# Chuanming-Liu/DAzimSurfTomo

Hardware: AMD Instinct MI355X
Metric: FMM traveltime fields/sec (256^2 grid, 16 periods) + LSQR SpMV HBM GB/s (higher is better)
Workload: dtype f32

## Files before the change

### dazimsurftomo_amd/__init__.py

```python
import ctypes as C

import numpy as np

from . import _lib
from ._lib import Geom, RefBox, build, load

RMAX = 129
PI_F32 = np.float32(3.1415926535898)


DAZIM_OK, DAZIM_E_SOURCE_OUTSIDE, DAZIM_E_RECEIVER_OUTSIDE, DAZIM_E_NNZ_OVERFLOW, DAZIM_E_BAD_ARG, DAZIM_E_ROOT_NOT_FOUND = 0, 1, 2, 4, 5, 6


class DazimError(RuntimeError):
    def __init__(self, code, msg):
        super().__init__(f"dazim error {code}: {msg}")
        self.code = code


def _is_torch(x):
    return type(x).__module__.startswith("torch")


def _ptr(x, dtype=None):
# ... 157 lines not shown
        kmax = len(tRc)
        if _is_torch(vel):
            import torch
            if lsen is None:
                lsen = torch.empty((nz - 1, kmax, nx * ny), dtype=torch.float32, device=vel.device)
        else:
            vel = np.ascontiguousarray(vel, np.float32)
            pv = np.ascontiguousarray(pv, np.float64)
            if lsen is None:
                lsen = np.zeros((nz - 1, kmax, nx * ny), np.float32)
        fn = self.lib.dazim_ti_kernels_sharded if sharded else self.lib.dazim_ti_kernels
        rc = fn(self._h, nx, ny, nz, _ptr(vel, np.float32), _ptr(depz), C.c_float(minthk), kmax, _ptr(tRc), _ptr(pv), _ptr(lsen))
        self._check(rc)
        return lsen

    def fmm_batch(self, nx, ny, goxd, gozd, dvxd, dvzd, pv, scx, scz, period_idx,
                  veln=None, ttn=None, ttnr=None, nstsr=None, boxes=None, status=None,
                  want_refined=True, keep_fields=False):
        g = geometry(nx, ny, goxd, gozd, dvxd, dvzd)
        kmax = pv.shape[0]
        nfield = int(scx.shape[0])
        if not _is_torch(pv):
            pv = np.ascontiguousarray(pv, np.float64)
            scx = np.ascontiguousarray(scx, np.float32)
            scz = np.ascontiguousarray(scz, np.float32)
            period_idx = np.ascontiguousarray(period_idx, np.int32)
            if ttn is None and not keep_fields:
                ttn = np.zeros((nfield, g.nnx, g.nnz), np.float32)
            if veln is None:
                veln = np.zeros((kmax, g.nnx, g.nnz), np.float32)
            if want_refined and ttnr is None:
                ttnr = np.zeros((nfield, RMAX, RMAX), np.float32)
                nstsr = np.zeros((nfield, RMAX, RMAX), np.int32)
            if boxes is None:
                boxes = (RefBox * max(nfield, 1))()
            if status is None:
                status = np.zeros(nfield, np.int32)
        if keep_fields:
            ttn = None
        bptr = None
        if boxes is not None:
            bptr = C.c_void_p(boxes.data_ptr()) if _is_torch(boxes) else C.cast(boxes, C.c_void_p)
        rc = self.lib.dazim_fmm_batch(self._h, nx, ny, C.c_float(goxd), C.c_float(gozd), C.c_float(dvxd),
                                      C.c_float(dvzd), kmax, _ptr(pv), nfield, _ptr(scx), _ptr(scz),
                                      _ptr(period_idx), _ptr(veln), _ptr(ttn), _ptr(ttnr), _ptr(nstsr),
                                      bptr, _ptr(status))
        out = dict(geom=g, veln=veln, ttn=ttn, ttnr=ttnr, nstsr=nstsr, boxes=boxes, status=status, rc=rc)
        if rc:
            err = DazimError(rc, self.lib.dazim_last_error(self._h).decode())
            err.partial = out
            raise err
        return out

    def rays_build_G(self, nx, ny, goxd, gozd, dvxd, dvzd, vels, fields, scx, scz, period_idx, field_of_ray,
                     rcx, rcz, sen, kernel_idx=None, tpred=None, lsen=None):
        nz = vels.shape[0]
        kmax = fields["veln"].shape[0]
        nfield = int(scx.shape[0])
        nray = int(rcx.shape[0])
        if tpred is None:
            if _is_torch(rcx):
                import torch
                tpred = torch.empty(nray, dtype=torch.float32, device=rcx.device)
            else:
                tpred = np.zeros(nray, np.float32)
        boxes = fields["boxes"]
        bptr = C.c_void_p(boxes.data_ptr()) if _is_torch(boxes) else C.cast(boxes, C.c_void_p)
        h = C.c_void_p()
        nnz = C.c_int64(0)
        nb = C.c_int(0)
        args = [self._h, nx, ny, nz, C.c_float(goxd), C.c_float(gozd), C.c_float(dvxd),
                C.c_float(dvzd), kmax, _ptr(vels, np.float32), nfield, _ptr(scx), _ptr(scz),
                _ptr(period_idx), _ptr(kernel_idx), _ptr(fields["veln"]), _ptr(fields["ttn"]),
                _ptr(fields["ttnr"]), _ptr(fields["nstsr"]), bptr, C.c_int64(nray),
                _ptr(field_of_ray), _ptr(rcx), _ptr(rcz), _ptr(sen[0]), _ptr(sen[1]), _ptr(sen[2])]
        tail = [_ptr(tpred), C.byref(h), C.byref(nnz), C.byref(nb)]
        if lsen is None:
            rc = self.lib.dazim_rays_build_G(*args, *tail)
        else:
            rc = self.lib.dazim_rays_build_G_joint(*args, _ptr(lsen, np.float32), *tail)
        self._check(rc)
        n = (nx - 2) * (ny - 2) * (nz - 1) * (1 if lsen is None else 3)
        return SparseMatrix(self, h, nray, n, nnz.value), tpred, nb.value

    def rays_build_G_maps(self, nx, ny, goxd, gozd, dvxd, dvzd, fields, scx, scz, period_idx, field_of_ray, rcx, rcz,
                          azim=False, tpred=None):
        kmax = fields["veln"].shape[0]
        nfield = int(scx.shape[0])
        nray = int(rcx.shape[0])
        if tpred is None:
            if _is_torch(rcx):
                import torch
                tpred = torch.empty(nray, dtype=torch.float32, device=rcx.device)
            else:
                tpred = np.zeros(nray, np.float32)
        boxes = fields["boxes"]
        bptr = C.c_void_p(boxes.data_ptr()) if _is_torch(boxes) else C.cast(boxes, C.c_void_p)
        h = C.c_void_p()
        nnz = C.c_int64(0)
        nb = C.c_int(0)
        rc = self.lib.dazim_rays_build_G_maps(self._h, nx, ny, C.c_float(goxd), C.c_float(gozd), C.c_float(dvxd), C.c_float(dvzd),
                                              kmax, int(bool(azim)), nfield, _ptr(scx), _ptr(scz), _ptr(period_idx),
                                              _ptr(fields["veln"]), _ptr(fields["ttn"]), _ptr(fields["ttnr"]), _ptr(fields["nstsr"]),
                                              bptr, C.c_int64(nray), _ptr(field_of_ray), _ptr(rcx), _ptr(rcz), _ptr(tpred),
                                              C.byref(h), C.byref(nnz), C.byref(nb))
        self._check(rc)
        n = (nx - 2) * (ny - 2) * kmax * (3 if azim else 1)
        return SparseMatrix(self, h, nray, n, nnz.value), tpred, nb.value

    def phase_map_update(self, nx, ny, pv, dm, minc, maxc, azim):
        kmax = pv.shape[0]
        assert pv.size == kmax * nx * ny and pv.flags.c_contiguous
        ncell = (nx - 2) * (ny - 2)
        nblock = 3 if azim else 1
        assert pv.dtype == np.float64 and dm.dtype == np.float32 and len(dm) == ncell * kmax * nblock
        a1 = np.zeros((kmax, ny - 2, nx - 2), np.float32) if azim else None
        a2 = np.zeros((kmax, ny - 2, nx - 2), np.float32) if azim else None
        st = np.zeros((nblock, kmax, 3), np.float32)
        self._check(self.lib.dazim_phase_map_update(self._h, nx, ny, kmax, int(bool(azim)), _ptr(pv), _ptr(dm), C.c_float(minc),
                                                    C.c_float(maxc), _ptr(a1), _ptr(a2), _ptr(st)))
        return a1, a2, st

    def vs_kernels(self, vel, sen, skern=None):
        nz, ny, nx = vel.shape
        kmax = sen[0].shape[1]
        if skern is None:
            if _is_torch(vel):
                import torch
                skern = torch.empty((nz, kmax, nx * ny), dtype=torch.float64, device=vel.device)
            else:
                skern = np.zeros((nz, kmax, nx * ny), np.float64)
        if not _is_torch(vel):
            vel = np.ascontiguousarray(vel, np.float32)
            sen = [np.ascontiguousarray(s, np.float64) for s in sen]
        self._check(self.lib.dazim_vs_kernels(self._h, nx, ny, nz, kmax, _ptr(vel, np.float32), _ptr(sen[0], np.float64),
                                              _ptr(sen[1], np.float64), _ptr(sen[2], np.float64), _ptr(skern, np.float64)))
        return skern

    def column_lsq(self, nx, ny, nlay, kern, rhs, wdat=None, smooth=0.0, damp=0.0, x=None):
        kmax = kern.shape[1]
        nrhs = rhs.shape[0]
        fp32 = str(kern.dtype).endswith("float32")
        if x is None:
            if _is_torch(rhs):
                import torch
                x = torch.empty((nrhs, nlay, ny - 2, nx - 2), dtype=torch.float32, device=rhs.device)
            else:
                x = np.zeros((nrhs, nlay, ny - 2, nx - 2), np.float32)
        if not _is_torch(rhs):
            kern = np.ascontiguousarray(kern)
            rhs = np.ascontiguousarray(rhs, np.float32)
            wdat = None if wdat is None else np.ascontiguousarray(wdat, np.float32)
        ne = C.c_int(0)
        st = np.zeros((nrhs, kmax, 2), np.float32)
        self._check(self.lib.dazim_column_lsq(self._h, nx, ny, int(nlay), kmax, int(fp32), _ptr(kern, np.float32 if fp32 else np.float64),
                                              nrhs, _ptr(rhs, np.float32), _ptr(wdat, np.float32), C.c_float(smooth), C.c_float(damp),
                                              _ptr(x, np.float32), C.byref(ne), _ptr(st)))
        return x, ne.value, st

# ... 264 lines not shown
```

### dazimsurftomo_amd/csrc/rays.hip

```cpp
#include <cmath>
#include <chrono>
#include <unistd.h>

#include "dazim_internal.h"

#include <rocprim/device/device_scan.hpp>
#include <rocprim/device/device_radix_sort.hpp>

namespace {

#ifdef DZ_RAYS_MARK
#define RAYS_MARK(i) asm volatile("; MARK " #i ::: "memory")
#else
#define RAYS_MARK(i)
#endif

constexpr int GDX = 5, GDZ = 5;
constexpr int RM = DAZIM_RMAX;
constexpr float EARTH = 6371.0f;
constexpr float FTOL = 1e-4f;

struct RayArgs {
  dazim_geom g;
  int nx, ny, nz, kmax;
// ... 151 lines not shown
    }
  return biv;
}

__global__ void k_row_kernels(long n, int kmax, long ncol, const float *__restrict__ vels, const double *__restrict__ svs,
                              const double *__restrict__ svp, const double *__restrict__ srho, double *__restrict__ out) {
  const long i = (long)blockIdx.x * blockDim.x + threadIdx.x;
  if (i >= n) return;
  const long k = i / (kmax * ncol), c = i % ncol;
  out[i] = dz_row_kernel(vels[k * ncol + c], svs[i], svp[i], srho[i]);
}

__global__ void k_ray_keys(long nray, const int *__restrict__ field, const float *__restrict__ scx, const float *__restrict__ scz,
                           const float *__restrict__ rcx, const float *__restrict__ rcz, float inv_dmax, int dbits,
                           unsigned *__restrict__ keys, unsigned *__restrict__ iota, const int *__restrict__ order) {
  const long i = (long)blockIdx.x * blockDim.x + threadIdx.x;
  if (i >= nray) return;
  const int f = field[i];
  const float dx = scx[f] - rcx[i], dz = (scz[f] - rcz[i]) * __sinf(rcx[i]);
  const float d = sqrtf(dx * dx + dz * dz) * inv_dmax;
  const unsigned dmaxq = (1u << dbits) - 1u;
  unsigned q = d >= 1.0f ? dmaxq : (unsigned)(d * (float)dmaxq);
  keys[i] = ((unsigned)(order ? order[f] : f) << dbits) | (dmaxq - q);
  iota[i] = (unsigned)i;
}

constexpr int GP_COUNT = 8, GP_EMIT = 16;
constexpr int RAYS_MINW = 4;
constexpr int RPW_MAX = 64 / GP_COUNT;
__device__ __forceinline__ void cbar() { asm volatile("" ::: "memory"); }

template <bool EMIT, bool AZIM, bool TILED, bool MAP>
__global__ __launch_bounds__(64, AZIM ? 2 : RAYS_MINW) void rays_kernel(RayArgs A_) {
  using ArgP = const __attribute__((address_space(4))) RayArgs *;
  auto launder = [](ArgP p) {
    int z;
    asm volatile("v_mov_b32 %0, 0" : "=v"(z));
    return (ArgP)((const __attribute__((address_space(4))) char *)p + __builtin_amdgcn_readfirstlane(z));
  };
  ArgP Ap = launder((ArgP)__builtin_amdgcn_kernarg_segment_ptr());
#define A (*Ap)
#define RAYS_ARGS_FRESH Ap = launder(Ap)
  constexpr int GP = EMIT ? GP_EMIT : GP_COUNT;
  constexpr int RPW = 64 / GP;
  constexpr int LPR = 16 / GP;
  constexpr int LSTEP = 4 / LPR;
  constexpr unsigned GMASK = (1u << GP) - 1u;
  extern __shared__ __attribute__((aligned(16))) unsigned short s_lists[];
  dazim_geom g;
  g.nvx = A.g.nvx; g.nvz = A.g.nvz; g.nnx = A.g.nnx; g.nnz = A.g.nnz;
  g.gox = A.g.gox; g.goz = A.g.goz; g.dnx = A.g.dnx; g.dnz = A.g.dnz; g.dvx = A.g.dvx; g.dvz = A.g.dvz;
  const int lane = threadIdx.x, grp = lane / GP, gl = lane & (GP - 1);
  const int lm = gl & 3, l0 = gl >> 2;
  const int nnx = g.nnx, nnz = g.nnz, nvx = g.nvx, nvz = g.nvz, ldf = nvz + 2, nf = ldf * (nvx + 2);
  constexpr int NG = AZIM ? 3 : 1;
  const unsigned nvx_magic = A.nvx_magic;
  const int LC = A.lcap;
  unsigned short *s_list = s_lists + (size_t)grp * LC;
  float *gfdm = A.fdm_scratch + ((size_t)blockIdx.x * RPW + grp) * nf * NG;
  float *gfdmc = gfdm + nf, *gfdms = gfdm + 2 * nf;
  const float gox = g.gox, goz = g.goz, dnx = g.dnx, dnz = g.dnz, dvx = g.dvx, dvz = g.dvz;
  const double rdnx = A.r_dnx, rdnz = A.r_dnz, rdnxr = A.r_dnxr, rdnzr = A.r_dnzr, rdvx = A.r_dvx, rdvz = A.r_dvz;
  const unsigned gmask_shift = grp * GP;
  const long nquad = (A.nray + RPW - 1) / RPW;
  const int nxcd = (gridDim.x % 8 == 0) ? 8 : 1;
  unsigned *qcnt = A.qcount + (EMIT ? 8 : 0);
  int chunk = (int)(blockIdx.x % nxcd);
  int traced = 0;
  for (;;) {
    RAYS_ARGS_FRESH;
    long quad = -1;
    if (lane == 0) {
      for (int tried = 0; tried < nxcd; tried++) {
        const long lo = nquad * chunk / nxcd, hi = nquad * (chunk + 1) / nxcd;
        const long b = lo < hi ? (long)atomicAdd(&qcnt[chunk], 1u) : hi;
        if (lo + b < hi) {
          quad = lo + b;
          break;
        }
        if (!EMIT && A.sweeps > 1 && lo < hi && b < (hi - lo) * A.sweeps) {
          quad = lo + b % (hi - lo);
          break;
        }
        chunk = (chunk + 1) % nxcd;
      }
    }
    quad = ((long)__shfl((int)(quad >> 32), 0) << 32) | (unsigned)__shfl((int)quad, 0);
    chunk = __shfl(chunk, 0);
    if (quad < 0) break;
    const long slot = quad * RPW + grp;
    if (!EMIT && A.defer_mark) {
      if (!A.defer_mark[quad]) continue;
      if (A.fdone) {
        const int fq = slot < A.nray ? A.field[A.perm ? (long)A.perm[slot] : slot] : -1;
        const int st = fq >= 0 ? __hip_atomic_load(A.fdone + fq, __ATOMIC_ACQUIRE, __HIP_MEMORY_SCOPE_AGENT) : 1;
        if (__ballot(st != 1) != 0) continue;
        __builtin_amdgcn_fence(__ATOMIC_ACQUIRE, "agent");
      }
      if (A.max_quads > 0 && traced >= A.max_quads) break;
      int mine = 0;
      if (lane == 0) mine = __hip_atomic_exchange(A.defer_mark + quad, 0, __ATOMIC_RELAXED, __HIP_MEMORY_SCOPE_AGENT);
      mine = __shfl(mine, 0);
      if (!mine) continue;
      traced++;
      if (lane == 0) atomicAdd(&A.qcount[18], 1u);
    }
    if (slot >= A.nray) continue;
    const long ray = A.perm ? (long)A.perm[slot] : slot;
    const int f = A.field[ray];
    const float scx = A.scx[f], scz = A.scz[f], rcx = A.rcx[ray], rcz = A.rcz[ray];
    const float *veln = A.veln + (size_t)(A.period[f] - 1) * nnx * nnz;
    const float *ttn = TILED ? A.ttn + (size_t)(A.tslot ? A.tslot[f] : f) * A.fstride : A.ttn + (size_t)f * nnx * nnz;
    const int tsh = TILED ? A.tsh : 0;
    auto tnode = [&](int x0, int z0) -> float {
      return TILED ? ttn[dz_tile_x(x0, tsh) + dz_tile_z(z0)] : ttn[(size_t)x0 * nnz + z0];
    };
    const float *ttnr = A.ttnr + (size_t)f * RM * RM;
    const int *nstsr = A.nstsr + (size_t)f * RM * RM;
    const dazim_refbox bx = A.boxes[f];
    const int saved = EMIT ? A.nlist[ray] : -1;
    if (saved < 0)
      for (int i = gl; i < nf * NG; i += GP) gfdm[i] = 0.0f;
    cbar();
    int status = 0, rb = 0;
    if (!EMIT) {
      int irx = (int)divr(rcx - gox, rdnx) + 1, irz = (int)divr(rcz - goz, rdnz) + 1;
      if (irx < 1 || irx > nnx || irz < 1 || irz > nnz) status = DAZIM_E_RECEIVER_OUTSIDE;
      if (!status) {
        if (irx == nnx) irx--;
        if (irz == nnz) irz--;
        const int isx = (int)divr(scx - gox, rdnx) + 1, isz = (int)divr(scz - goz, rdnz) + 1;
        float sred = ((scx - rcx) * EARTH) * ((scx - rcx) * EARTH);
        const float e2 = (scz - rcz) * EARTH * dz_sinf(rcx);
        sred = sqrtf(sred + e2 * e2);
        bool sw = sred < A.dplh;
        if (isx == irx && isz == irz) sw = true;
        float trr;
        if (sw) {
          const float vs = bilin_cell(g, veln, isx, isz, scx, scz, rdnx, rdnz);
          const float vr = bilin_cell(g, veln, irx, irz, rcx, rcz, rdnx, rdnz);
          trr = 2.0f * sred / (vs + vr);
        } else {
          const float drx = (rcx - gox) - (float)(irx - 1) * dnx;
          const float drz = (rcz - goz) - (float)(irz - 1) * dnz;
          trr = 0.0f;
#pragma unroll
          for (int k = 1; k <= 2; k++)
#pragma unroll
            for (int l = 1; l <= 2; l++) {
              const float produ = (1.0f - fabsf(divr((float)(l - 1) * dnz - drz, rdnz))) *
                                  (1.0f - fabsf(divr((float)(k - 1) * dnx - drx, rdnx)));
              trr = trr + tnode(irx - 2 + k, irz - 2 + l) * produ;
            }
        }
        if (gl == 0) A.dsurf[ray] = trr;
      }
    }
    const float goxr = bx.goxr, gozr = bx.gozr, dnxr = bx.dnxr, dnzr = bx.dnzr;
    const int nnxr = bx.nnxr, nnzr = bx.nnzr;
    const int isx = (int)divr(scx - goxr, rdnxr) + 1, isz = (int)divr(scz - gozr, rdnzr) + 1;
    const float dpl = 0.5f * A.dplh;
    int ipx = (int)divr(rcx - gox, rdnx) + 1, ipz = (int)divr(rcz - goz, rdnz) + 1;
    if (ipx < 1 || ipx >= nnx || ipz < 1 || ipz >= nnz) status = DAZIM_E_RECEIVER_OUTSIDE;
    if (!status && saved < 0) {
      float x0 = rcx, z0 = rcz;
      float sinx0 = dz_sinf(x0);
      int sw = 0;
      float sred = ((scx - x0) * EARTH) * ((scx - x0) * EARTH);
      float e2 = (scz - z0) * EARTH * sinx0;
      sred = sqrtf(sred + e2 * e2);
      if (sred < 2.0f * dpl) sw = 1;
      int ipxr = (int)divr(rcx - goxr, rdnxr) + 1, ipzr = (int)divr(rcz - gozr, rdnzr) + 1;
      auto in_refined = [&](int px, int pz) -> int {
        if (px < 1 || px >= nnxr || pz < 1 || pz >= nnzr) return 0;
        const int *sp = nstsr + (size_t)(px - 1) * RM + (pz - 1);
        if (sp[0] != 0 || sp[1] != 0) return 0;
        if (sp[RM] != 0 || sp[RM + 1] != 0) return 0;
        return 1;
      };
      int igref = in_refined(ipxr, ipzr);
      if (sw == 0 && igref == 1 && ipxr == isx && ipzr == isz) sw = 1;
      const bool keep_pts = !EMIT && A.pts != nullptr && gl == 0;
      float2 *rp = A.pts ? A.pts + (size_t)ray * A.pcap : nullptr;
      int np = 1;
      if (keep_pts) {
        rp[0] = make_float2(rcx, rcz);
        if (sw == 1) { if (A.pcap > 1) rp[1] = make_float2(scx, scz); np = 2; }
      }
      int cbx = -100, cbz = -100;
      float acc[LPR], accc[LPR], accs[LPR];
#pragma unroll
      for (int q = 0; q < LPR; q++) acc[q] = accc[q] = accs[q] = 0.0f;
      auto flush = [&]() {
        if (cbx > -100) {
#pragma unroll
          for (int q = 0; q < LPR; q++) {
            const int fi = (cbx + lm) * ldf + (cbz + l0 + q * LSTEP);
            gfdm[fi] = acc[q];
            if (AZIM) { gfdmc[fi] = accc[q]; gfdms[fi] = accs[q]; }
          }
        }
      };
      float tc00, tc01, tc10, tc11, tr00 = 0.0f, tr01 = 0.0f, tr10 = 0.0f, tr11 = 0.0f;
      auto load_corner_times = [&]() {
        if (TILED) {
          const int x0 = dz_tile_x(ipx - 1, tsh), x1 = dz_tile_x(ipx, tsh), z0 = dz_tile_z(ipz - 1), z1 = dz_tile_z(ipz);
          tc00 = ttn[x0 + z0]; tc01 = ttn[x0 + z1]; tc10 = ttn[x1 + z0]; tc11 = ttn[x1 + z1];
        } else {
          const float *t = ttn + (size_t)(ipx - 1) * nnz + (ipz - 1);
          tc00 = t[0]; tc01 = t[1]; tc10 = t[nnz]; tc11 = t[nnz + 1];
        }
      };
      auto load_refined_corner_times = [&]() {
        if (ipxr >= 1 && ipxr < nnxr && ipzr >= 1 && ipzr < nnzr) {
          const float *u = ttnr + (size_t)(ipxr - 1) * RM + (ipzr - 1);
          tr00 = u[0]; tr01 = u[1]; tr10 = u[RM]; tr11 = u[RM + 1];
        }
      };
      load_corner_times();
      load_refined_corner_times();
      bool carry = false;
      float rdc[LPR];
#pragma unroll
      for (int q = 0; q < LPR; q++) rdc[q] = 0.0f;
      float fart = __builtin_inff();
      int nnx_in = 0, nnz_in = 0;
      const long maxrp = (long)nnx * nnz;
      for (long j = 1; j <= maxrp; j++) {
        if (sw == 1) break;
        RAYS_MARK(0);
        float dtx, dtz;
        if (igref == 1) {
          dtx = tr10 - tr00;
          dtx = dtx + tr11 - tr01;
          dtx = divr(dtx, A.r_e2dnxr);
          dtz = tr01 - tr00;
          dtz = dtz + tr11 - tr10;
          dtz = dtz / (2.0f * EARTH * sinx0 * dnzr);
        } else {
          dtx = tc10 - tc00;
          dtx = dtx + tc11 - tc01;
          dtx = divr(dtx, A.r_e2dnx);
          dtz = tc01 - tc00;
          dtz = dtz + tc11 - tc10;
          dtz = dtz / (2.0f * EARTH * sinx0 * dnz);
        }
        const float rd1 = sqrtf(dtx * dtx + dtz * dtz);
        float x1 = x0 - dpl * dtx / (EARTH * rd1);
        float z1 = z0 - dpl * dtz / (EARTH * sinx0 * rd1);
        RAYS_MARK(1);
// ... 72 lines not shown
        RAYS_MARK(6);
        float drx, drz;
        if (__builtin_expect(__ballot(!carry) != 0, 0)) {
          drx = (x0 - gox) - (float)(ipxo - 1) * dnx;
          drz = (z0 - goz) - (float)(ipzo - 1) * dnz;
          const float vel = vel_at(g, veln, ipxo, ipzo, drx, drz, rdnx, rdnz);
          drx = (x0 - gox) - (float)(ivxo - 1) * dvx;
          drz = (z0 - goz) - (float)(ivzo - 1) * dvz;
          const float vi = basis1(divr(drx, rdvx), lm);
#pragma unroll
          for (int q = 0; q < LPR; q++) rdc[q] = vi * basis1(divr(drz, rdvz), l0 + q * LSTEP) / (vel * vel);
          if (A.plain_step == 0) {
            fart = (float)((RM - 1) / 8 + 1) * fmaxf(dnx, dnz);
            nnx_in = nnx;
            nnz_in = nnz;
          }
        }
        RAYS_MARK(7);
        int ivxt = ivxo, ivzt = ivzo;
        bool endsame = false;
        for (int k = 1; k <= nhp; k++) {
          if (k > 1) {
            const int cp = (k == 2) ? chp0 : chp1;
            if (cp == 1) ivxt = ivx;
            else if (cp == 2) ivzt = ivz;
          }
          const float vrk = (k == 1) ? vr0 : (k == 2 ? vr1 : vr2);
          const float vrp = (k == 2) ? vr0 : vr1;
          const float rigz = z0 + vrk * (z1 - z0);
          const float rigx = x0 + vrk * (x1 - x0);
          const int ipxt = (int)divr(rigx - gox, rdnx) + 1, ipzt = (int)divr(rigz - goz, rdnz) + 1;
          endsame = rigx == x1 && rigz == z1 && ipxt == ipx && ipzt == ipz && ivxt == ivx && ivzt == ivz;
          drx = (rigx - gox) - (float)(ipxt - 1) * dnx;
          drz = (rigz - goz) - (float)(ipzt - 1) * dnz;
          const bool inner = ipxt >= 1 && ipxt < nnx_in && ipzt >= 1 && ipzt < nnz_in;
          endsame = endsame && inner;
          float vel;
          if (__builtin_expect(__ballot(!inner) == 0, 1)) vel = vel_at_interior(g, veln, ipxt, ipzt, drx, drz, rdnx, rdnz);
          else vel = vel_at(g, veln, ipxt, ipzt, drx, drz, rdnx, rdnz);
          drx = (rigx - gox) - (float)(ivxt - 1) * dvx;
          drz = (rigz - goz) - (float)(ivzt - 1) * dvz;
          const float vi = basis1(divr(drx, rdvx), lm);
          float wi[LPR];
#pragma unroll
          for (int q = 0; q < LPR; q++) wi[q] = basis1(divr(drz, rdvz), l0 + q * LSTEP);
          const float dinc = (k == 1) ? vrk * dpl : (vrk - vrp) * dpl;
          const int nbx = ivxt - 1, nbz = ivzt - 1;
          RAYS_MARK(8);
          if (nbx != cbx || nbz != cbz) {
            flush();
            cbar();
            cbx = nbx;
            cbz = nbz;
#pragma unroll
            for (int q = 0; q < LPR; q++) {
              const int fi = (cbx + lm) * ldf + (cbz + l0 + q * LSTEP);
              acc[q] = gfdm[fi];
              if (AZIM) { accc[q] = gfdmc[fi]; accs[q] = gfdms[fi]; }
            }
          }
          RAYS_MARK(9);
#pragma unroll
          for (int q = 0; q < LPR; q++) {
            const float rdc1 = vi * wi[q] / (vel * vel);
            const float rdc2 = rdc[q];
            rdc[q] = rdc1;
            float r1 = -(rdc1 + rdc2) * dinc / 2.0f;
            acc[q] = r1 + acc[q];
            if (AZIM) {
              r1 = -(rdc1 * c2psi + rdc2 * c2psi) * dinc / 2.0f;
              accc[q] = r1 + accc[q];
              r1 = -(rdc1 * s2psi + rdc2 * s2psi) * dinc / 2.0f;
              accs[q] = r1 + accs[q];
            }
          }
        }
        RAYS_MARK(10);
        carry = endsame;
        x0 = x1;
        z0 = z1;
        sinx0 = sinx1;
      RAYS_MARK(11);
      }
      flush();
      if (keep_pts) A.npts[ray] = np <= A.pcap ? np : -1;
    }
    cbar();
    if (!EMIT && gl == 0) {
      if (A.pts && status) A.npts[ray] = 0;
      A.status[ray] = status;
      A.rbflag[ray] = rb;
    }
    int nlist = 0;
    if (saved >= 0) {
      nlist = saved;
      const size_t o = (size_t)ray * A.LK, ov = o * NG;
      for (int i = gl; i < nlist; i += GP) {
        const int c = A.lcell[o + i];
        const int jj = (int)__umulhi((unsigned)c, nvx_magic) + 1, kk = c - (jj - 1) * nvx + 1;
        s_list[i] = (unsigned short)c;
        gfdm[kk * ldf + jj] = A.lval[ov + i];
        if (AZIM) {
          gfdmc[kk * ldf + jj] = A.lval[ov + A.LK + i];
          gfdms[kk * ldf + jj] = A.lval[ov + 2 * A.LK + i];
        }
      }
    } else if (!status) {
      for (int base = 0; base < nvz * nvx; base += GP) {
        const int c = base + gl;
        bool keep = false;
        if (c < nvz * nvx) {
          const int jj = (int)__umulhi((unsigned)c, nvx_magic) + 1, kk = c - (jj - 1) * nvx + 1;
          keep = fabsf(gfdm[kk * ldf + jj]) >= FTOL;
        }
        const unsigned m = (unsigned)((__ballot(keep) >> gmask_shift) & GMASK);
        const int pos = nlist + __popc(m & ((1u << gl) - 1u));
        if (keep && pos < LC) s_list[pos] = (unsigned short)c;
        nlist += __popc(m);
      }
    }
    cbar();
    if (!EMIT) {
      const size_t o = (size_t)ray * A.LK, ov = o * NG;
      if (nlist <= A.LK)
        for (int i = gl; i < nlist; i += GP) {
          const int c = s_list[i];
          const int jj = (int)__umulhi((unsigned)c, nvx_magic) + 1, kk = c - (jj - 1) * nvx + 1;
          A.lcell[o + i] = (unsigned short)c;
          A.lval[ov + i] = gfdm[kk * ldf + jj];
          if (AZIM) {
            A.lval[ov + A.LK + i] = gfdmc[kk * ldf + jj];
            A.lval[ov + 2 * A.LK + i] = gfdms[kk * ldf + jj];
          }
        }
      if (gl == 0) A.nlist[ray] = (status || nlist <= A.LK) ? (status ? 0 : nlist) : -1;
    }
    const size_t ncol = (size_t)A.nx * A.ny;
    const int kslot = A.kidx[f] - 1;
    long cnt = 0;
    const long rstart = EMIT ? A.rowptr[ray] : 0;
    const int nparpi = nvx * nvz * (A.nz - 1);
    const int nlay = MAP ? 1 : A.nz - 1;
    const int bstride = MAP ? A.kmax * nvx * nvz : nparpi;
    const int poff = MAP ? (A.period[f] - 1) * nvx * nvz : 0;
    const bool lovf = nlist > LC;
    const int ntot = lovf ? nvz * nvx : nlist;
    long cntd = 0;
    int jjL = 1, kkL = 1;
    if (A.dense) {
      int clast = -1;
      if (!lovf) {
        if (nlist > 0) clast = s_list[nlist - 1];
      } else {
        for (int base = ((nvz * nvx - 1) / GP) * GP; base >= 0 && clast < 0; base -= GP) {
          const int c = base + gl;
          bool k2 = false;
          if (c < nvz * nvx) {
            const int jj = (int)__umulhi((unsigned)c, nvx_magic) + 1, kk = c - (jj - 1) * nvx + 1;
            k2 = fabsf(gfdm[kk * ldf + jj]) >= FTOL;
          }
          const unsigned m2 = (unsigned)((__ballot(k2) >> gmask_shift) & GMASK);
          if (m2) clast = base + (31 - __clz(m2));
        }
      }
      if (clast >= 0) { jjL = (int)__umulhi((unsigned)clast, nvx_magic) + 1; kkL = clast - (jjL - 1) * nvx + 1; }
    }
    constexpr int RC = 8;
    const bool rowcache = !lovf && ntot <= RC * GP && (MAP || A.skern != nullptr) && !A.dense;
    if (rowcache) {
      int sidx[RC], cbase[RC], fidx[RC];
#pragma unroll
      for (int i = 0; i < RC; i++) {
        const int li = i * GP + gl;
        const int c = li < ntot ? (int)s_list[li] : 0;
        const int jj = (int)__umulhi((unsigned)c, nvx_magic) + 1, kk = c - (jj - 1) * nvx + 1;
        sidx[i] = jj * (nvx + 2) + kk;
        cbase[i] = (jj - 1) * nvx + kk;
        fidx[i] = kk * ldf + jj;
      }
      for (int blk = 0; blk < NG; blk++) {
        float fdv[RC];
        const float *fsrc = blk == 0 ? gfdm : (blk == 1 ? gfdmc : gfdms);
#pragma unroll
        for (int i = 0; i < RC; i++) fdv[i] = (i * GP + gl < ntot) ? fsrc[fidx[i]] : 0.0f;
        for (int k = 1; k <= nlay; k++) {
          const size_t sk = ((size_t)(k - 1) * A.kmax + kslot) * ncol;
          const int nk = blk * bstride + poff + (k - 1) * nvz * nvx;
#pragma unroll
          for (int i = 0; i < RC; i++) {
            if (i * GP >= ntot) break;
            const bool cell = i * GP + gl < ntot;
            float rowv = 0.0f;
            bool keep = false;
            if (cell) {
              if (MAP) rowv = fdv[i];
              else if (blk == 0) rowv = (float)(A.skern[sk + sidx[i]] * (double)fdv[i]);
              else rowv = A.lsen[sk + sidx[i]] * fdv[i];
              keep = A.keep_small ? (rowv != 0.0f) : (fabsf(rowv) > FTOL);
            }
            const unsigned m = (unsigned)((__ballot(keep) >> gmask_shift) & GMASK);
            if (EMIT && keep) {
              const long pos = rstart + cnt + __popc(m & ((1u << gl) - 1u));
              A.val[pos] = rowv;
              A.col[pos] = nk + cbase[i] - 1;
            }
            cnt += __popc(m);
          }
        }
      }
    } else
    for (int blk = 0; blk < NG; blk++)
      for (int k = 1; k <= nlay; k++) {
        for (int base = 0; base < ntot; base += GP) {
          const int li = base + gl;
          bool keep = false, keepd = false;
          float rowv = 0.0f;
          int nn = 0;
          bool cell = li < ntot;
          int c = 0;
          if (cell) c = lovf ? li : s_list[li];
          const int jj = (int)__umulhi((unsigned)c, nvx_magic) + 1, kk = c - (jj - 1) * nvx + 1;
          if (cell && lovf) cell = fabsf(gfdm[kk * ldf + jj]) >= FTOL;
          if (cell && MAP) {
            rowv = (blk == 0 ? gfdm : (blk == 1 ? gfdmc : gfdms))[kk * ldf + jj];
            keep = A.keep_small ? (rowv != 0.0f) : (fabsf(rowv) > FTOL);
            nn = blk * bstride + poff + (jj - 1) * nvx + kk;
          } else if (cell) {
            const size_t si = ((size_t)(k - 1) * A.kmax + kslot) * ncol + (size_t)jj * (nvx + 2) + kk;
            if (blk == 0) {
              const float fd = gfdm[kk * ldf + jj];
              double r;
              if (A.skern) {
                r = A.skern[si] * (double)fd;
              } else {
                const float v = A.vels[((size_t)(k - 1) * A.ny + jj) * A.nx + kk];
                const float coe_a = (2.0947f - 0.8206f * 2 * v + 0.2683f * 3 * (v * v) - 0.0251f * 4 * (v * v * v));
                const float vpft = 0.9409f + 2.0947f * v - 0.8206f * (v * v) + 0.2683f * (v * v * v) - 0.0251f * (v * v * v * v);
                const float coe_rho = coe_a * (1.6612f - 0.4721f * 2 * vpft + 0.0671f * 3 * (vpft * vpft) -
                                               0.0043f * 4 * (vpft * vpft * vpft) + 0.000106f * 5 * (vpft * vpft * vpft * vpft));
                r = (A.svp[si] * (double)coe_a + A.srho[si] * (double)coe_rho + A.svs[si]) * (double)fd;
              }
              rowv = (float)r;
              if (A.dense) {
                const float vL = A.vels[((size_t)(k - 1) * A.ny + jjL) * A.nx + kkL];
                const float caL = (2.0947f - 0.8206f * 2 * vL + 0.2683f * 3 * (vL * vL) - 0.0251f * 4 * (vL * vL * vL));
                const float vpL = 0.9409f + 2.0947f * vL - 0.8206f * (vL * vL) + 0.2683f * (vL * vL * vL) - 0.0251f * (vL * vL * vL * vL);
                const float crL = caL * (1.6612f - 0.4721f * 2 * vpL + 0.0671f * 3 * (vpL * vpL) -
                                         0.0043f * 4 * (vpL * vpL * vpL) + 0.000106f * 5 * (vpL * vpL * vpL * vpL));
                const double rd = (A.svp[si] * (double)caL + A.srho[si] * (double)crL + A.svs[si]) * (double)fd;
                keepd = (float)rd != 0.0f;
                if (EMIT && A.dense == 1) rowv = (float)rd;
              }
            } else {
              rowv = A.lsen[si] * (blk == 1 ? gfdmc : gfdms)[kk * ldf + jj];
              keepd = rowv != 0.0f;
            }
            keep = A.keep_small ? (rowv != 0.0f) : (fabsf(rowv) > FTOL);
            if (EMIT && A.dense == 1) keep = keepd;
            nn = blk * bstride + (k - 1) * nvz * nvx + (jj - 1) * nvx + kk;
          }
          if (!EMIT && A.dense == 2) cntd += __popc((unsigned)((__ballot(keepd) >> gmask_shift) & GMASK));
          const unsigned m = (unsigned)((__ballot(keep) >> gmask_shift) & GMASK);
          if (EMIT && keep) {
            const long pos = rstart + cnt + __popc(m & ((1u << gl) - 1u));
            A.val[pos] = rowv;
            A.col[pos] = nn - 1;
          }
          cnt += __popc(m);
        }
      }
    if (!EMIT && gl == 0) {
      A.count[ray] = cnt;
      if (A.dense == 2) A.countd[ray] = cntd;
      if (lovf) atomicAdd(&A.qcount[16], 1u);
      if (!status && nlist > A.LK) atomicAdd(&A.qcount[17], 1u);
    }
  }
}
#undef A
#undef RAYS_ARGS_FRESH

struct RayBuild {
  dazim_ctx *ctx;
  int nx = 0, ny = 0, nz = 0, kmax = 0, nfield = 0;
  float goxd = 0, gozd = 0, dvxd = 0, dvzd = 0;
  const float *vels = nullptr, *scx = nullptr, *scz = nullptr, *veln = nullptr, *ttn = nullptr, *ttnr = nullptr, *rcx = nullptr, *rcz = nullptr;
  const float *lsen = nullptr;
  const int *period = nullptr, *kidx = nullptr, *nstsr = nullptr, *field = nullptr;
  const dazim_refbox *boxes = nullptr;
  const double *svs = nullptr, *svp = nullptr, *srho = nullptr;
  int64_t nray = 0;
  float *dsurf = nullptr;
  dazim_csr **G = nullptr;
  int64_t *nnz_out = nullptr;
  int *n_boundary = nullptr;
  bool map = false, azim = false;
  struct StreamSwap {
    dazim_ctx *c; hipStream_t main; bool on = false;
    void restore() { if (on) { c->stream = main; on = false; } }
    ~StreamSwap() {
      if (on) (void)hipStreamSynchronize(c->stream);
      restore();
    }
  } swap;
  struct {
    DzBuf<float> vels, scx, scz, veln, ttn, ttnr, rcx, rcz, dsurf, lsen;
    DzBuf<int> period, kidx, nstsr, field;
    DzBuf<dazim_refbox> boxes;
    DzBuf<double> svs, svp, srho;
  } d;
  struct Arrays {
    dazim_ctx *c; int64_t *rp = nullptr; float *v = nullptr; int *cl = nullptr; int64_t nnz = 0, cap_nnz = 0; bool keep = false;
    ~Arrays() { if (!keep) { dz_big_put(c, rp); dz_big_put(c, v); dz_big_put(c, cl); } }
  } arrays, arrays_d;
  dazim_geom g;
  bool joint = false, tiled = false, overlap = false, twin = false;
  size_t nn = 0, nr = 0, ncol = 0, nk = 0, nr1 = 0, lds = 0;
  int64_t res_rows = 0, res_nnz = 0;
  long nwg = 0;
  double overlap_tail_s = 0.0;
  RayArgs A;
  explicit RayBuild(dazim_ctx *c) : ctx(c), swap{c, c ? c->stream : nullptr}, arrays{c}, arrays_d{c} {}
  int check() {
// ... 121 lines not shown
      if ((rc = dz_scratch(ctx, "rays.pts", nr1 * (size_t)A.pcap, &A.pts))) return rc;
      if ((rc = dz_scratch(ctx, "rays.npts", nr1, &A.npts))) return rc;
      DZ_HIP(hipMemsetAsync(A.npts, 0, nr1 * 4, ctx->stream));
    }
    ctx->ksec["rays.path_cap"] = A.pcap;
    ctx->ksec["rays.path_rays"] = A.pts ? (double)nray : 0.0;
    twin = dz_opt(ctx, "rays.dense_twin", 0) != 0 && !A.keep_small;
    A.dense = twin ? 2 : 0;
    A.countd = nullptr;
    if (twin) {
      if ((rc = dz_scratch(ctx, "rays.countd", (size_t)(nray + 1), &A.countd))) return rc;
      DZ_HIP(hipMemsetAsync(A.countd, 0, (size_t)(nray + 1) * 8, ctx->stream));
    }
    if ((rc = dz_scratch(ctx, "rays.nlist", nr1, &A.nlist))) return rc;
    if ((rc = dz_scratch(ctx, "rays.lcell", nr1 * A.LK, &A.lcell))) return rc;
    if ((rc = dz_scratch(ctx, "rays.lval", nr1 * A.LK * (joint ? 3 : 1), &A.lval))) return rc;
    res_rows = (int64_t)g.nvx * g.nvz * (map ? kmax : nz - 1) * (joint ? 3 : 1);
    res_nnz = (map ? 5 : 7) * res_rows;
    if (dz_opt(ctx, "csr.reserve_rows", 0) > res_rows) res_rows = dz_opt(ctx, "csr.reserve_rows", 0);
    if (dz_opt(ctx, "csr.reserve_nnz", 0) > res_nnz) res_nnz = dz_opt(ctx, "csr.reserve_nnz", 0);
    if ((rc = dz_big_get(ctx, (size_t)(nray + res_rows + 1), &arrays.rp))) return rc;
    A.dsurf = d.dsurf.dev;
    A.rowptr = (const long *)arrays.rp; A.val = nullptr; A.col = nullptr;
    return 0;
  }
  template <int I> static const void *kernel_no() { return (const void *)rays_kernel<(I & 8) != 0, (I & 4) != 0, (I & 2) != 0, (I & 1) != 0>; }
  const void *kern(bool emit) const {
    static const void *const tab[16] = {kernel_no<0>(),  kernel_no<1>(),  kernel_no<2>(),  kernel_no<3>(), kernel_no<4>(),  kernel_no<5>(),
                                        kernel_no<6>(),  kernel_no<7>(),  kernel_no<8>(),  kernel_no<9>(), kernel_no<10>(), kernel_no<11>(),
                                        kernel_no<12>(), kernel_no<13>(), kernel_no<14>(), kernel_no<15>()};
    return tab[(emit ? 8 : 0) + (joint ? 4 : 0) + (tiled ? 2 : 0) + (map ? 1 : 0)];
  }
  int launch(bool emit, const RayArgs &R, long nwg_) {
    RayArgs args = R;
    void *params[] = {&args};
    DZ_HIP(hipLaunchKernel(kern(emit), dim3((unsigned)nwg_), dim3(64), params, lds, ctx->stream));
    return 0;
  }
  int launch_shape() {
    lds = (size_t)A.lcap * 2 * RPW_MAX + 16;
    DZ_HIP(hipFuncSetAttribute(kern(false), hipFuncAttributeMaxDynamicSharedMemorySize, (int)lds));
    DZ_HIP(hipFuncSetAttribute(kern(true), hipFuncAttributeMaxDynamicSharedMemorySize, (int)lds));
    int per_cu = (int)(160 * 1024 / (lds + 256));
    {
      int occ = 0;
      const void *kf = kern(false);
      if (hipOccupancyMaxActiveBlocksPerMultiprocessor(&occ, kf, 64, lds) == hipSuccess && occ > 0 && occ < per_cu) per_cu = occ;
    }
    if (per_cu > 16) per_cu = 16;
    if (per_cu < 1) return dz_fail(ctx, DAZIM_E_BAD_ARG, "inversion grid too large for the LDS cell lists");
    if (dz_opt(ctx, "rays.wg_per_cu", 0) > 0 && dz_opt(ctx, "rays.wg_per_cu", 0) < per_cu) per_cu = dz_opt(ctx, "rays.wg_per_cu", 0);
    nwg = (long)ctx->num_cu * per_cu;
    if (nwg > (nray + RPW_MAX - 1) / RPW_MAX) nwg = (nray + RPW_MAX - 1) / RPW_MAX;
    if (nwg >= 8) nwg -= nwg % 8;
    if (nwg < 1) nwg = 1;
    return dz_scratch(ctx, "rays.fdm", (size_t)nwg * RPW_MAX * (g.nvx + 2) * (g.nvz + 2) * (joint ? 3 : 1), &A.fdm_scratch);
  }
  int sort_rays() {
    int rc;
    A.perm = nullptr;
    if (nray >= 64 && nray < (1ll << 32) && dz_opt(ctx, "rays.sort", 1) != 0) {
      int fbits = 1;
      while ((1ll << fbits) < nfield) fbits++;
      const int dbits = 32 - fbits > 12 ? 12 : 32 - fbits;
      if (dbits >= 4) {
        unsigned *k0, *k1, *v0, *v1;
        if ((rc = dz_scratch(ctx, "rays.sortbuf", (size_t)nray * 4 + 16, &k0))) return rc;
        k1 = k0 + nray; v0 = k1 + nray; v1 = v0 + nray;
        const float ex = (float)g.nnx * g.dnx, ez = (float)g.nnz * g.dnz;
        const float inv_dmax = 1.0f / sqrtf(ex * ex + ez * ez);
        hipLaunchKernelGGL(k_ray_keys, dim3((unsigned)((nray + 255) / 256)), dim3(256), 0, ctx->stream, (long)nray, d.field.dev, d.scx.dev,
                           d.scz.dev, d.rcx.dev, d.rcz.dev, inv_dmax, dbits, k0, v0, overlap ? A.tslot : (const int *)nullptr);
        size_t tb = 0;
        DZ_HIP(rocprim::radix_sort_pairs(nullptr, tb, k0, k1, v0, v1, (size_t)nray, 0, fbits + dbits, ctx->stream));
        void *tmp;
        if ((rc = dz_scratch(ctx, "rays.sorttmp", tb + 256, &tmp))) return rc;
        DZ_HIP(rocprim::radix_sort_pairs(tmp, tb, k0, k1, v0, v1, (size_t)nray, 0, fbits + dbits, ctx->stream));
        A.perm = v1;
      }
    }
    if ((rc = dz_scratch(ctx, "rays.qcount", 32, &A.qcount))) return rc;
    DZ_HIP(hipMemsetAsync(A.qcount, 0, 128, ctx->stream));
    if (overlap) {
      const size_t nq = (size_t)((nray + RPW_MAX - 1) / RPW_MAX) + 8;
      if ((rc = dz_scratch(ctx, "rays.defer", nq, &A.defer_mark))) return rc;
      DZ_HIP(hipMemsetAsync(A.defer_mark, 0, nq * 4, ctx->stream));
    }
    return 0;
  }
  int count_pass() { return nray > 0 ? launch(false, A, nwg) : 0; }
  int count_passes_beside_eikonal() {
    int rc;
    const auto t_poll0 = std::chrono::steady_clock::now();
    auto fmm_over = [&]() {
      const bool over = hipEventQuery(ctx->ev_f1) == hipSuccess;
      if (!over) (void)hipGetLastError();
      return over;
    };
    if (ctx->fields.hprog && ctx->fields.total_tasks > 0) {
      const unsigned slack = ctx->fields.nwg / 4 + 8 * 16;
      const unsigned total = ctx->fields.total_tasks;
      const unsigned want = total > slack ? total - slack : 0;
      for (;;) {
        unsigned have = 0;
        for (int c = 0; c < 8; c++) have += ctx->fields.hprog[c];
        if (have >= want || fmm_over()) break;
        if (std::chrono::steady_clock::now() - t_poll0 > std::chrono::seconds(120)) break;
        usleep(50);
      }
// ... 198 lines not shown
```

Measured before the change: 55700.

## Track ray bounding box to skip full-grid scratch zeroing and list scans

Before, the per-ray scratch sensitivity grid was zeroed in full for every ray and scanned in full to build the nonzero cell list. Now the kernel tracks the min/max box of visited cells with LDS atomics and scans and clears only that box. The scratch is zeroed once at allocation, and the layout is transposed to row-major z so the box scans read contiguous memory. On the EMIT pass with saved lists, row-cache values come straight from lval and only the touched cells are cleared. This adds an optional nwg cap and richer error info, and relies on every path restoring zeros correctly.

```diff
diff --git a/dazimsurftomo_amd/__init__.py b/dazimsurftomo_amd/__init__.py
--- a/dazimsurftomo_amd/__init__.py
+++ b/dazimsurftomo_amd/__init__.py
@@ -233,6 +233,12 @@
             raise err
         return out
 
+    def _check_rays(self, rc, tpred, nnz, nb):
+        if rc:
+            err = DazimError(rc, self.lib.dazim_last_error(self._h).decode())
+            err.partial = {"tpred": tpred, "nnz": nnz.value, "n_boundary": nb.value}
+            raise err
+
     def rays_build_G(self, nx, ny, goxd, gozd, dvxd, dvzd, vels, fields, scx, scz, period_idx, field_of_ray,
                      rcx, rcz, sen, kernel_idx=None, tpred=None, lsen=None):
         nz = vels.shape[0]
@@ -260,7 +266,7 @@
             rc = self.lib.dazim_rays_build_G(*args, *tail)
         else:
             rc = self.lib.dazim_rays_build_G_joint(*args, _ptr(lsen, np.float32), *tail)
-        self._check(rc)
+        self._check_rays(rc, tpred, nnz, nb)
         n = (nx - 2) * (ny - 2) * (nz - 1) * (1 if lsen is None else 3)
         return SparseMatrix(self, h, nray, n, nnz.value), tpred, nb.value
 
@@ -285,7 +291,7 @@
                                               _ptr(fields["veln"]), _ptr(fields["ttn"]), _ptr(fields["ttnr"]), _ptr(fields["nstsr"]),
                                               bptr, C.c_int64(nray), _ptr(field_of_ray), _ptr(rcx), _ptr(rcz), _ptr(tpred),
                                               C.byref(h), C.byref(nnz), C.byref(nb))
-        self._check(rc)
+        self._check_rays(rc, tpred, nnz, nb)
         n = (nx - 2) * (ny - 2) * kmax * (3 if azim else 1)
         return SparseMatrix(self, h, nray, n, nnz.value), tpred, nb.value
 
diff --git a/dazimsurftomo_amd/csrc/rays.hip b/dazimsurftomo_amd/csrc/rays.hip
--- a/dazimsurftomo_amd/csrc/rays.hip
+++ b/dazimsurftomo_amd/csrc/rays.hip
@@ -227,13 +227,17 @@
   g.gox = A.g.gox; g.goz = A.g.goz; g.dnx = A.g.dnx; g.dnz = A.g.dnz; g.dvx = A.g.dvx; g.dvz = A.g.dvz;
   const int lane = threadIdx.x, grp = lane / GP, gl = lane & (GP - 1);
   const int lm = gl & 3, l0 = gl >> 2;
-  const int nnx = g.nnx, nnz = g.nnz, nvx = g.nvx, nvz = g.nvz, ldf = nvz + 2, nf = ldf * (nvx + 2);
+  const int nnx = g.nnx, nnz = g.nnz, nvx = g.nvx, nvz = g.nvz;
+  const int ldf = nvx + 2, nf = ldf * (nvz + 2);
   constexpr int NG = AZIM ? 3 : 1;
   const unsigned nvx_magic = A.nvx_magic;
   const int LC = A.lcap;
   unsigned short *s_list = s_lists + (size_t)grp * LC;
   float *gfdm = A.fdm_scratch + ((size_t)blockIdx.x * RPW + grp) * nf * NG;
   float *gfdmc = gfdm + nf, *gfdms = gfdm + 2 * nf;
+  __shared__ int s_rngs[RPW][4];
+  int *s_rng = s_rngs[grp];
+  constexpr int RC = 8;
   const float gox = g.gox, goz = g.goz, dnx = g.dnx, dnz = g.dnz, dvx = g.dvx, dvz = g.dvz;
   const double rdnx = A.r_dnx, rdnz = A.r_dnz, rdnxr = A.r_dnxr, rdnzr = A.r_dnzr, rdvx = A.r_dvx, rdvz = A.r_dvz;
   const unsigned gmask_shift = grp * GP;
@@ -294,8 +298,7 @@
     const int *nstsr = A.nstsr + (size_t)f * RM * RM;
     const dazim_refbox bx = A.boxes[f];
     const int saved = EMIT ? A.nlist[ray] : -1;
-    if (saved < 0)
-      for (int i = gl; i < nf * NG; i += GP) gfdm[i] = 0.0f;
+    if (saved < 0 && gl < 4) s_rng[gl] = gl < 2 ? 0x7fffffff : -1;
     cbar();
     int status = 0, rb = 0;
     if (!EMIT) {
@@ -370,7 +373,7 @@
         if (cbx > -100) {
 #pragma unroll
           for (int q = 0; q < LPR; q++) {
-            const int fi = (cbx + lm) * ldf + (cbz + l0 + q * LSTEP);
+            const int fi = (cbz + l0 + q * LSTEP) * ldf + (cbx + lm);
             gfdm[fi] = acc[q];
             if (AZIM) { gfdmc[fi] = accc[q]; gfdms[fi] = accs[q]; }
           }
@@ -549,9 +552,13 @@
             cbar();
             cbx = nbx;
             cbz = nbz;
+            __hip_atomic_fetch_min(s_rng + 0, nbx, __ATOMIC_RELAXED, __HIP_MEMORY_SCOPE_WORKGROUP);
+            __hip_atomic_fetch_min(s_rng + 1, nbz, __ATOMIC_RELAXED, __HIP_MEMORY_SCOPE_WORKGROUP);
+            __hip_atomic_fetch_max(s_rng + 2, nbx, __ATOMIC_RELAXED, __HIP_MEMORY_SCOPE_WORKGROUP);
+            __hip_atomic_fetch_max(s_rng + 3, nbz, __ATOMIC_RELAXED, __HIP_MEMORY_SCOPE_WORKGROUP);
 #pragma unroll
             for (int q = 0; q < LPR; q++) {
-              const int fi = (cbx + lm) * ldf + (cbz + l0 + q * LSTEP);
+              const int fi = (cbz + l0 + q * LSTEP) * ldf + (cbx + lm);
               acc[q] = gfdm[fi];
               if (AZIM) { accc[q] = gfdmc[fi]; accs[q] = gfdms[fi]; }
             }
@@ -588,33 +595,35 @@
       A.status[ray] = status;
       A.rbflag[ray] = rb;
     }
+    auto usual = [&](int n) { return n <= LC && n <= RC * GP && (MAP || A.skern != nullptr) && !A.dense; };
     int nlist = 0;
     if (saved >= 0) {
       nlist = saved;
       const size_t o = (size_t)ray * A.LK, ov = o * NG;
+      const bool viaslot = !usual(saved);
       for (int i = gl; i < nlist; i += GP) {
         const int c = A.lcell[o + i];
-        const int jj = (int)__umulhi((unsigned)c, nvx_magic) + 1, kk = c - (jj - 1) * nvx + 1;
         s_list[i] = (unsigned short)c;
-        gfdm[kk * ldf + jj] = A.lval[ov + i];
-        if (AZIM) {
-          gfdmc[kk * ldf + jj] = A.lval[ov + A.LK + i];
-          gfdms[kk * ldf + jj] = A.lval[ov + 2 * A.LK + i];
+        if (viaslot) {
+          const int jj = (int)__umulhi((unsigned)c, nvx_magic) + 1, kk = c - (jj - 1) * nvx + 1;
+          gfdm[jj * ldf + kk] = A.lval[ov + i];
+          if (AZIM) {
+            gfdmc[jj * ldf + kk] = A.lval[ov + A.LK + i];
+            gfdms[jj * ldf + kk] = A.lval[ov + 2 * A.LK + i];
+          }
         }
       }
     } else if (!status) {
-      for (int base = 0; base < nvz * nvx; base += GP) {
-        const int c = base + gl;
-        bool keep = false;
-        if (c < nvz * nvx) {
-          const int jj = (int)__umulhi((unsigned)c, nvx_magic) + 1, kk = c - (jj - 1) * nvx + 1;
-          keep = fabsf(gfdm[kk * ldf + jj]) >= FTOL;
-        }
-        const unsigned m = (unsigned)((__ballot(keep) >> gmask_shift) & GMASK);
-        const int pos = nlist + __popc(m & ((1u << gl) - 1u));
-        if (keep && pos < LC) s_list[pos] = (unsigned short)c;
-        nlist += __popc(m);
-      }
+      const int kk0 = max(s_rng[0], 1), kk1 = min(s_rng[2] + 3, nvx), jj0 = max(s_rng[1], 1), jj1 = min(s_rng[3] + 3, nvz);
+      for (int jj = jj0; jj <= jj1; jj++)
+        for (int kb = kk0; kb <= kk1; kb += GP) {
+          const int kk = kb + gl;
+          const bool keep = kk <= kk1 && fabsf(gfdm[jj * ldf + kk]) >= FTOL;
+          const unsigned m = (unsigned)((__ballot(keep) >> gmask_shift) & GMASK);
+          const int pos = nlist + __popc(m & ((1u << gl) - 1u));
+          if (keep && pos < LC) s_list[pos] = (unsigned short)((jj - 1) * nvx + kk - 1);
+          nlist += __popc(m);
+        }
     }
     cbar();
     if (!EMIT) {
@@ -624,10 +633,10 @@
           const int c = s_list[i];
           const int jj = (int)__umulhi((unsigned)c, nvx_magic) + 1, kk = c - (jj - 1) * nvx + 1;
           A.lcell[o + i] = (unsigned short)c;
-          A.lval[ov + i] = gfdm[kk * ldf + jj];
+          A.lval[ov + i] = gfdm[jj * ldf + kk];
           if (AZIM) {
-            A.lval[ov + A.LK + i] = gfdmc[kk * ldf + jj];
-            A.lval[ov + 2 * A.LK + i] = gfdms[kk * ldf + jj];
+            A.lval[ov + A.LK + i] = gfdmc[jj * ldf + kk];
+            A.lval[ov + 2 * A.LK + i] = gfdms[jj * ldf + kk];
           }
         }
       if (gl == 0) A.nlist[ray] = (status || nlist <= A.LK) ? (status ? 0 : nlist) : -1;
@@ -654,7 +663,7 @@
           bool k2 = false;
           if (c < nvz * nvx) {
             const int jj = (int)__umulhi((unsigned)c, nvx_magic) + 1, kk = c - (jj - 1) * nvx + 1;
-            k2 = fabsf(gfdm[kk * ldf + jj]) >= FTOL;
+            k2 = fabsf(gfdm[jj * ldf + kk]) >= FTOL;
           }
           const unsigned m2 = (unsigned)((__ballot(k2) >> gmask_shift) & GMASK);
           if (m2) clast = base + (31 - __clz(m2));
@@ -662,8 +671,7 @@
       }
       if (clast >= 0) { jjL = (int)__umulhi((unsigned)clast, nvx_magic) + 1; kkL = clast - (jjL - 1) * nvx + 1; }
     }
-    constexpr int RC = 8;
-    const bool rowcache = !lovf && ntot <= RC * GP && (MAP || A.skern != nullptr) && !A.dense;
+    const bool rowcache = usual(nlist);
     if (rowcache) {
       int sidx[RC], cbase[RC], fidx[RC];
 #pragma unroll
@@ -673,13 +681,14 @@
         const int jj = (int)__umulhi((unsigned)c, nvx_magic) + 1, kk = c - (jj - 1) * nvx + 1;
         sidx[i] = jj * (nvx + 2) + kk;
         cbase[i] = (jj - 1) * nvx + kk;
-        fidx[i] = kk * ldf + jj;
+        fidx[i] = jj * ldf + kk;
       }
       for (int blk = 0; blk < NG; blk++) {
         float fdv[RC];
         const float *fsrc = blk == 0 ? gfdm : (blk == 1 ? gfdmc : gfdms);
-#pragma unroll
-        for (int i = 0; i < RC; i++) fdv[i] = (i * GP + gl < ntot) ? fsrc[fidx[i]] : 0.0f;
+        const float *lsrc = A.lval + ((size_t)ray * NG + blk) * A.LK;
+#pragma unroll
+        for (int i = 0; i < RC; i++) fdv[i] = (i * GP + gl < ntot) ? (saved >= 0 ? lsrc[i * GP + gl] : fsrc[fidx[i]]) : 0.0f;
         for (int k = 1; k <= nlay; k++) {
           const size_t sk = ((size_t)(k - 1) * A.kmax + kslot) * ncol;
           const int nk = blk * bstride + poff + (k - 1) * nvz * nvx;
@@ -717,15 +726,15 @@
           int c = 0;
           if (cell) c = lovf ? li : s_list[li];
           const int jj = (int)__umulhi((unsigned)c, nvx_magic) + 1, kk = c - (jj - 1) * nvx + 1;
-          if (cell && lovf) cell = fabsf(gfdm[kk * ldf + jj]) >= FTOL;
+          if (cell && lovf) cell = fabsf(gfdm[jj * ldf + kk]) >= FTOL;
           if (cell && MAP) {
-            rowv = (blk == 0 ? gfdm : (blk == 1 ? gfdmc : gfdms))[kk * ldf + jj];
+            rowv = (blk == 0 ? gfdm : (blk == 1 ? gfdmc : gfdms))[jj * ldf + kk];
             keep = A.keep_small ? (rowv != 0.0f) : (fabsf(rowv) > FTOL);
             nn = blk * bstride + poff + (jj - 1) * nvx + kk;
           } else if (cell) {
             const size_t si = ((size_t)(k - 1) * A.kmax + kslot) * ncol + (size_t)jj * (nvx + 2) + kk;
             if (blk == 0) {
-              const float fd = gfdm[kk * ldf + jj];
+              const float fd = gfdm[jj * ldf + kk];
               double r;
               if (A.skern) {
                 r = A.skern[si] * (double)fd;
@@ -749,7 +758,7 @@
                 if (EMIT && A.dense == 1) rowv = (float)rd;
               }
             } else {
-              rowv = A.lsen[si] * (blk == 1 ? gfdmc : gfdms)[kk * ldf + jj];
+              rowv = A.lsen[si] * (blk == 1 ? gfdmc : gfdms)[jj * ldf + kk];
               keepd = rowv != 0.0f;
             }
             keep = A.keep_small ? (rowv != 0.0f) : (fabsf(rowv) > FTOL);
@@ -766,6 +775,23 @@
           cnt += __popc(m);
         }
       }
+    cbar();
+    if (saved < 0) {
+      const int x0 = max(s_rng[0], 0), x1 = min(s_rng[2] + 3, nvx + 1), z0 = max(s_rng[1], 0), z1 = min(s_rng[3] + 3, nvz + 1);
+      for (int z = z0; z <= z1; z++)
+        for (int x = x0 + gl; x <= x1; x += GP) {
+          gfdm[z * ldf + x] = 0.0f;
+          if (AZIM) { gfdmc[z * ldf + x] = 0.0f; gfdms[z * ldf + x] = 0.0f; }
+        }
+    } else if (!rowcache) {
+      for (int i = gl; i < nlist; i += GP) {
+        const int c = s_list[i];
+        const int jj = (int)__umulhi((unsigned)c, nvx_magic) + 1, kk = c - (jj - 1) * nvx + 1;
+        gfdm[jj * ldf + kk] = 0.0f;
+        if (AZIM) { gfdmc[jj * ldf + kk] = 0.0f; gfdms[jj * ldf + kk] = 0.0f; }
+      }
+    }
+    cbar();
     if (!EMIT && gl == 0) {
       A.count[ray] = cnt;
       if (A.dense == 2) A.countd[ray] = cntd;
@@ -993,9 +1019,15 @@
     if (dz_opt(ctx, "rays.wg_per_cu", 0) > 0 && dz_opt(ctx, "rays.wg_per_cu", 0) < per_cu) per_cu = dz_opt(ctx, "rays.wg_per_cu", 0);
     nwg = (long)ctx->num_cu * per_cu;
     if (nwg > (nray + RPW_MAX - 1) / RPW_MAX) nwg = (nray + RPW_MAX - 1) / RPW_MAX;
+    if (dz_opt(ctx, "rays.nwg", 0) > 0 && dz_opt(ctx, "rays.nwg", 0) < nwg) nwg = dz_opt(ctx, "rays.nwg", 0);
     if (nwg >= 8) nwg -= nwg % 8;
     if (nwg < 1) nwg = 1;
-    return dz_scratch(ctx, "rays.fdm", (size_t)nwg * RPW_MAX * (g.nvx + 2) * (g.nvz + 2) * (joint ? 3 : 1), &A.fdm_scratch);
+    const size_t nslot = (size_t)nwg * RPW_MAX * (g.nvx + 2) * (g.nvz + 2) * (joint ? 3 : 1);
+    int rc;
+    if ((rc = dz_scratch(ctx, "rays.fdm", nslot, &A.fdm_scratch))) return rc;
+    DZ_HIP(hipMemsetAsync(A.fdm_scratch, 0, nslot * sizeof(float), ctx->stream));
+    ctx->ksec["rays.nwg"] = (double)nwg;
+    return 0;
   }
   int sort_rays() {
     int rc;
```

Result: faster. 56790, median of 6 (+2.0%).
